# jakepoz/rnnt

Hardware: AMD Instinct MI355X
Metric: RNN-T joint+loss fwd+bwd lattice cells/s (B*T*U/s) (higher is better)
Workload: dtype f32(f16x2); 1 GPU; cfg2: B=32,T=1000,U=200,H=512,V=1024 fp32-class (f16x2 arithmetic) joint+loss fwd+bwd; enc_layout=contiguous (B,T,H), global_batch=32, per_gpu_batch=32, parallelism=dp1, cells_BTU1=6432000

## Files before the change

### rnnt_amd/csrc/common.hpp

```cpp
#pragma once
#include <hip/hip_runtime.h>
#include <stdint.h>

typedef float f32x16 __attribute__((ext_vector_type(16)));
typedef float f32x4 __attribute__((ext_vector_type(4)));

#define RNNT_NEG_INF (-__builtin_inff())
#ifdef RNNT_ABLATE
#define RNNT_XP(flags, bit) ((flags) & (bit))
#else
#define RNNT_XP(flags, bit) (0)
#endif
#define RNNT_LOG2E 1.4426950408889634f

#ifdef RNNT_VMCNT0
#define RNNT_VMCNT(n) "s_waitcnt vmcnt(0)"
#else
#define RNNT_VMCNT(n) "s_waitcnt vmcnt(" #n ")"
#endif

__device__ __forceinline__ long skew_index(int b, int t, int u, int D, int U1)
{
    return ((long)b * D + (t + u)) * U1 + u;
}

__device__ __forceinline__ int len_t(const int32_t *logit_lens, int b, int T)
{
    const int v = logit_lens[b];
    return v < 1 ? 1 : (v > T ? T : v);
}
__device__ __forceinline__ int len_u(const int32_t *target_lens, int b, int U1)
{
    const int v = target_lens[b];
    return v < 0 ? 0 : (v > U1 - 1 ? U1 - 1 : v);
}

__device__ __forceinline__ void len_tu_uniform(const int32_t *logit_lens, const int32_t *target_lens, int b, int T, int U1,
                                               int &Tb, int &Ub)
{
    int x, y;
    const int32_t *pl = logit_lens + b, *pt = target_lens + b;
    asm volatile("s_load_dword %0, %2, 0x0\n\ts_load_dword %1, %3, 0x0\n\ts_waitcnt lgkmcnt(0)"
                 : "=&s"(x), "=&s"(y) : "s"(pl), "s"(pt) : "memory");
    Tb = x < 1 ? 1 : (x > T ? T : x);
    Ub = y < 0 ? 0 : (y > U1 - 1 ? U1 - 1 : y);
}

__device__ __forceinline__ float fast_tanh(float x)
{
    float e = __builtin_amdgcn_exp2f(x * (2.0f * RNNT_LOG2E));
    return 1.0f - 2.0f * __builtin_amdgcn_rcpf(e + 1.0f);
}

typedef float f32x2_t __attribute__((ext_vector_type(2)));
__device__ __forceinline__ f32x2_t fast_tanh2(f32x2_t x)
{
    const f32x2_t a = x * (2.0f * RNNT_LOG2E);
    f32x2_t e = {__builtin_amdgcn_exp2f(a[0]), __builtin_amdgcn_exp2f(a[1])};
    e += 1.0f;
    const f32x2_t r = {__builtin_amdgcn_rcpf(e[0]), __builtin_amdgcn_rcpf(e[1])};
    return 1.0f - 2.0f * r;
}
__device__ __forceinline__ f32x4 fast_tanh_sum4(f32x4 e, f32x4 p)
{
    const f32x2_t lo = fast_tanh2(__builtin_shufflevector(e, e, 0, 1) + __builtin_shufflevector(p, p, 0, 1));
    const f32x2_t hi = fast_tanh2(__builtin_shufflevector(e, e, 2, 3) + __builtin_shufflevector(p, p, 2, 3));
    return f32x4{lo[0], lo[1], hi[0], hi[1]};
}

__device__ __forceinline__ float half_max(float v)
{
#pragma unroll
    for (int m = 16; m >= 1; m >>= 1) v = fmaxf(v, __shfl_xor(v, m, 64));
    return v;
}
__device__ __forceinline__ float half_sum(float v)
{
#pragma unroll
    for (int m = 16; m >= 1; m >>= 1) v += __shfl_xor(v, m, 64);
    return v;
}

template <int CTRL, int ROW_MASK>
__device__ __forceinline__ float dpp_mov(float old, float v)
{
    return __int_as_float(__builtin_amdgcn_update_dpp(__float_as_int(old), __float_as_int(v), CTRL, ROW_MASK, 0xf, false));
}
__device__ __forceinline__ float half_bcast(float v, int half)
{
    const float lo = __int_as_float(__builtin_amdgcn_readlane(__float_as_int(v), 31));
    const float hi = __int_as_float(__builtin_amdgcn_readlane(__float_as_int(v), 63));
    return half ? hi : lo;
}
__device__ __forceinline__ float half_max_dpp(float v, int half)
{
    asm volatile("s_nop 1\n\tv_max_f32_dpp %0, %0, %0 quad_perm:[1,0,3,2] row_mask:0xf bank_mask:0xf\n\t"
                 "s_nop 1\n\tv_max_f32_dpp %0, %0, %0 quad_perm:[2,3,0,1] row_mask:0xf bank_mask:0xf\n\t"
                 "s_nop 1\n\tv_max_f32_dpp %0, %0, %0 row_ror:4 row_mask:0xf bank_mask:0xf\n\t"
                 "s_nop 1\n\tv_max_f32_dpp %0, %0, %0 row_ror:8 row_mask:0xf bank_mask:0xf"
                 : "+v"(v));
    v = fmaxf(v, dpp_mov<0x142, 0xa>(RNNT_NEG_INF, v));
    return half_bcast(v, half);
}
__device__ __forceinline__ float half_sum_dpp(float v, int half)
{
    asm volatile("s_nop 1\n\tv_add_f32_dpp %0, %0, %0 quad_perm:[1,0,3,2] row_mask:0xf bank_mask:0xf\n\t"
                 "s_nop 1\n\tv_add_f32_dpp %0, %0, %0 quad_perm:[2,3,0,1] row_mask:0xf bank_mask:0xf\n\t"
                 "s_nop 1\n\tv_add_f32_dpp %0, %0, %0 row_ror:4 row_mask:0xf bank_mask:0xf\n\t"
                 "s_nop 1\n\tv_add_f32_dpp %0, %0, %0 row_ror:8 row_mask:0xf bank_mask:0xf"
                 : "+v"(v));
    v += dpp_mov<0x142, 0xa>(0.f, v);
    return v;
}

struct __attribute__((aligned(16))) CellCoef {
    float c1;
    float sb;
    float se;
    int y;
};
```

### rnnt_amd/csrc/x2.hip

```cpp
#include "kernels.hpp"

typedef __attribute__((ext_vector_type(8))) _Float16 f16x8;
typedef __attribute__((ext_vector_type(2))) _Float16 f16x2;
typedef __attribute__((ext_vector_type(4))) unsigned u32x4;
typedef __attribute__((ext_vector_type(2))) unsigned u32x2;
typedef __attribute__((ext_vector_type(4))) int i32x4;
typedef __attribute__((address_space(3))) void *lds_vptr;
typedef float f2 __attribute__((ext_vector_type(2)));

#ifdef RNNT_STAMPS
#define X2_CLOCK_STAMP(SLOT)                                                                                               \
    do {                                                                                                                   \
        if (a.debug && blockIdx.x == 0 && blockIdx.y == 0 && blockIdx.z == 0 && threadIdx.x == 0) {                        \
            unsigned long long t_, r_;                                                                                     \
            asm volatile("s_memtime %0\n\ts_memrealtime %1\n\ts_waitcnt lgkmcnt(0)" : "=s"(t_), "=s"(r_)::"memory");      \
            a.debug[SLOT] = t_; a.debug[(SLOT) + 1] = r_;                                                                  \
        }                                                                                                                  \
    } while (0)
#else
#define X2_CLOCK_STAMP(SLOT) do {} while (0)
#endif

#define X2_SH 16384.0f
#define X2_INV_SH (1.0f / 16384.0f)
// ... 1315 lines not shown
        __builtin_amdgcn_raw_ptr_buffer_load_lds(wrs, dst, 16, wvo, so, 1024, 0);
    };
    const int lds0 = (int)(size_t)(lds_vptr)s_dr;
    const int wb = lds0 + 16 * lane;

    f32x16 acc[4][4];
#pragma unroll
    for (int m = 0; m < 4; ++m)
#pragma unroll
        for (int n = 0; n < 4; ++n)
#pragma unroll
            for (int r = 0; r < 16; ++r) acc[m][n][r] = 0.f;

    AFrag ar[4];
    aload(ar[0], 0); aload(ar[1], 1); aload(ar[2], 2);
    wdma(0, 0); wdma(1, 1);
    int wsl = 0;
    for (int c0 = 0; c0 < VC; c0 += 4) {
#pragma unroll
        for (int j = 0; j < 4; ++j) {
            const int c = c0 + j;
            asm volatile(RNNT_VMCNT(10) ::: "memory");
            x2_lds_barrier();
            const int ws = wb + wsl * XR2_WSLOT;
            u32x4 bh[4], bm[4];
#pragma unroll
            for (int n = 0; n < 4; ++n) asm volatile("ds_read_b128 %0, %1 offset:%2" : "=v"(bh[n]) : "v"(ws), "n"(n * 1024));
            asm volatile("s_waitcnt lgkmcnt(0)" : "+v"(bh[0]), "+v"(bh[1]), "+v"(bh[2]), "+v"(bh[3]) :: "memory");
            AFrag &ac = ar[j], &an = ar[(j + 3) & 3];
            const int cn = c + 3;
            const int o = 8 * ((cn < VC ? cn : VC - 1) >> 1) + 2 * ((cn < VC ? cn : VC - 1) & 1);
#pragma unroll
            for (int m = 0; m < 4; ++m) {
#pragma unroll
                for (int n = 0; n < 4; ++n) {
                    acc[m][n] = x2_mfma(ac.h[m], bh[n], acc[m][n]);
                    if (m == 0) asm volatile("ds_read_b128 %0, %1 offset:%2" : "=v"(bm[n]) : "v"(ws), "n"(4096 + n * 1024));
                    if (n == 1) an.h[m] = arow[m][o];
                    if (n == 3) an.m[m] = arow[m][o + 4];
                    __builtin_amdgcn_sched_barrier(0);
                }
            }
#pragma unroll
            for (int m = 0; m < 4; ++m)
#pragma unroll
                for (int n = 0; n < 4; ++n) {
                    acc[m][n] = x2_mfma(ac.m[m], bh[n], acc[m][n]);
                    __builtin_amdgcn_sched_barrier(0);
                }
            asm volatile("s_waitcnt lgkmcnt(0)" : "+v"(bm[0]), "+v"(bm[1]), "+v"(bm[2]), "+v"(bm[3]) :: "memory");
#pragma unroll
            for (int m = 0; m < 4; ++m)
#pragma unroll
                for (int n = 0; n < 4; ++n) {
                    acc[m][n] = x2_mfma(ac.h[m], bm[n], acc[m][n]);
                    if (m == 3 && n == 0) wdma(c + 2, (wsl + 2) & 3);
                    __builtin_amdgcn_sched_barrier(0);
                }
            wsl = (wsl + 1) & 3;
        }
    }
    asm volatile("s_waitcnt vmcnt(0)" ::: "memory");
    if (!wlive) return;

    const int colg = 512 * hp + 4 * i;
    const bool colok = colg < H;
    f32x4 pr[8];
#pragma unroll
    for (int r7 = 0; r7 < 8; ++r7) {
        const int u = u0 + 8 * (r7 >> 2) + (r7 & 3) + 4 * half;
        pr[r7] = (u < U1 && colok) ? *(const f32x4 *)(a.pred + ((long)b * U1 + u) * H + colg) : f32x4{0.f, 0.f, 0.f, 0.f};
    }
    const float unscale = 4.0f * a.db_rescale * a.scales[1];
    const long BTH = (long)a.B * T * H, BUH = (long)a.B * U1 * H;
    auto dfac_q = [](f2 x) {
        const f2 av = x * (2.0f * RNNT_LOG2E);
        const f2 w = {__builtin_amdgcn_exp2f(-__builtin_fabsf(av[0])), __builtin_amdgcn_exp2f(-__builtin_fabsf(av[1]))};
        const f2 e1 = w + 1.0f;
        const f2 r = {__builtin_amdgcn_rcpf(e1[0]), __builtin_amdgcn_rcpf(e1[1])};
        return (w * r) * r;
    };
    f2 psum2[8][2];
#pragma unroll
    for (int k = 0; k < 8; ++k) { psum2[k][0] = f2{0.f, 0.f}; psum2[k][1] = f2{0.f, 0.f}; }
#pragma unroll
    for (int m = 0; m < 4; ++m)
#pragma unroll
        for (int rh = 0; rh < 2; ++rh) {
            const int t = t0 + 2 * m + rh;
            const f32x4 er = (t < T && colok) ? *(const f32x4 *)(a.enc + (long)b * a.enc_sb + (long)t * a.enc_st + colg) : f32x4{0.f, 0.f, 0.f, 0.f};
            f2 esum2[2] = {f2{0.f, 0.f}, f2{0.f, 0.f}};
#pragma unroll
            for (int r7 = 0; r7 < 8; ++r7)
#pragma unroll
                for (int qq = 0; qq < 2; ++qq) {
                    const f2 x = {er[2 * qq] + pr[r7][2 * qq], er[2 * qq + 1] + pr[r7][2 * qq + 1]};
                    const f2 av = {acc[m][2 * qq][rh * 8 + r7], acc[m][2 * qq + 1][rh * 8 + r7]};
                    const f2 d = av * dfac_q(x);
                    esum2[qq] += d;
                    psum2[r7][qq] += d;
                }
            f32x4 es = {unscale * esum2[0][0], unscale * esum2[0][1], unscale * esum2[1][0], unscale * esum2[1][1]};
#pragma unroll
            for (int q = 0; q < 4; ++q) es[q] += __shfl_xor(es[q], 32, 64);
            if (half == 0 && t < Tb && colok) *(f32x4 *)(a.slab_enc + (long)ub * BTH + ((long)b * T + t) * H + colg) = es;
        }
#pragma unroll
    for (int k = 0; k < 8; ++k) {
        const int u = u0 + 8 * (k >> 2) + (k & 3) + 4 * half;
        if (u < U1 && colok) {
            const f32x4 o = {unscale * psum2[k][0][0], unscale * psum2[k][0][1], unscale * psum2[k][1][0], unscale * psum2[k][1][1]};
            *(f32x4 *)(a.slab_pred + (long)tt * BUH + ((long)b * U1 + u) * H + colg) = o;
        }
    }
}

#define XZ2_WG_WAVES 4
__global__ __launch_bounds__(64 * XZ2_WG_WAVES) void k_x2_dead_rows(X3Args a, int ntt, int nub)
{
    const int lane = threadIdx.x & 63;
    const long wave = (long)blockIdx.x * XZ2_WG_WAVES + (threadIdx.x >> 6), nwave = (long)gridDim.x * XZ2_WG_WAVES;
    const long cells = (long)a.B * a.T * a.U1;
    const bool by_ks = a.dw_ksteps;
    const int sh = by_ks ? 4 : 2, per = 64 >> sh;
    const int *list = by_ks ? a.ks_list : a.grp_list;
    const long n = a.live_stats[by_ks ? 0 : 4];
    const int V4 = a.V / 4;
    const u32x4 z = {0u, 0u, 0u, 0u};
    for (long k = per * wave; k < n; k += per * nwave) {
        const long kk = k + (lane >> sh);
        int e = 0;
        bool dead = false;
        if (kk < n) {
            e = list[kk];
            const long c = ((long)e << sh) + (lane & ((1 << sh) - 1));
            if (c < cells) {
                const int u = (int)(c % a.U1);
                const long bt = c / a.U1;
                const int t = (int)(bt % a.T);
                const long b = bt / a.T;
                dead = a.tile_live[(b * ntt + t / XG2_BT_) * nub + u / XG2_BU_] == 0;
            }
        }
        unsigned long long m = __ballot(dead);
        for (; m; m &= m - 1) {
            const int r = __builtin_ctzll(m);
            u32x4 *row = (u32x4 *)(a.logits + (((long)__shfl(e, r, 64) << sh) + (r & ((1 << sh) - 1))) * a.V);
            for (int q = lane; q < V4; q += 64) row[q] = z;
        }
    }
}
void launch_x2_dead_rows(const X3Args &a, hipStream_t st)
{
    const long rounds = ((long)a.B * a.T * a.U1 + 63) / 64;
    const long want = (rounds + XZ2_WG_WAVES - 1) / XZ2_WG_WAVES, cap = (long)(a.n_cu > 0 ? a.n_cu : 256) * 8;
    const int ntt = (a.T + XG2_BT_ - 1) / XG2_BT_;
    hipLaunchKernelGGL(k_x2_dead_rows, dim3((unsigned)(want < cap ? want : cap)), dim3(64 * XZ2_WG_WAVES), 0, st, a, ntt, a.n_ublk16);
}

bool x2_dhidden_ok(int U1, int H, int V)
{
    return (long)((XG2_BT - 1) * (long)U1 + XG2_BU) * V * 4 < 0x7fffffffL && V % 128 == 0 && H % 128 == 0;
}

void launch_dhidden_x2(const X3Args &a, hipStream_t st)
{
    static bool attr_set[16] = {false};
    int dev = -1;
    if (hipGetDevice(&dev) != hipSuccess || dev < 0 || dev >= 16) dev = -1;
    const int lds = XG2_NW * XG2_WSLOT + 2 * XG2_XSLOT;
    if (dev < 0 || !attr_set[dev]) {
        (void)hipFuncSetAttribute((const void *)k_dhidden_x2<true, false>, hipFuncAttributeMaxDynamicSharedMemorySize, lds);
        (void)hipFuncSetAttribute((const void *)k_dhidden_x2<false, false>, hipFuncAttributeMaxDynamicSharedMemorySize, lds);
        (void)hipFuncSetAttribute((const void *)k_dhidden_x2<true, true>, hipFuncAttributeMaxDynamicSharedMemorySize, lds);
        (void)hipFuncSetAttribute((const void *)k_dhidden_x2<false, true>, hipFuncAttributeMaxDynamicSharedMemorySize, lds);
        if (dev >= 0) attr_set[dev] = true;
    }
    dim3 grid((unsigned)((long)a.n_ublk16 * ((a.T + XG2_BT - 1) / XG2_BT) * a.B));
    if (a.H < 512) hipLaunchKernelGGL((k_dhidden_x2<true, true>), grid, dim3(256), lds, st, a, 0);
    else hipLaunchKernelGGL((k_dhidden_x2<true, false>), grid, dim3(256), lds, st, a, 0);
    for (int hp = 1; hp * 512 < a.H; ++hp) {
        if (a.H - 512 * hp == 128) {
            dim3 gr(a.n_ublk16, ((a.T + XG2_BT - 1) / XG2_BT + 3) / 4, a.B);
            hipLaunchKernelGGL(k_dhidden_x2r, gr, dim3(256), XR2_NW * XR2_WSLOT, st, a, hp);
        }
        else if (a.H - 512 * hp < 512) hipLaunchKernelGGL((k_dhidden_x2<false, true>), grid, dim3(256), lds, st, a, hp);
        else hipLaunchKernelGGL((k_dhidden_x2<false, false>), grid, dim3(256), lds, st, a, hp);
    }
}

__global__ __launch_bounds__(256) void k_x2_make_ep(X3Args a)
{
    const int H = a.H, H4 = H / 4, KC = H / 16;
    const long n_enc = (long)a.B * a.T * H4, n_all = n_enc + (long)a.B * a.U1 * H4;
    const long idx = (long)blockIdx.x * 256 + threadIdx.x;
    bool big = false;
    if (idx < n_all) {
        const bool is_enc = idx < n_enc;
        const long j = is_enc ? idx : idx - n_enc;
        const long row = j / H4;
        const int h = (int)(j - row * H4) * 4;
        const int R = is_enc ? a.T : a.U1;
        const int b = (int)(row / R), r = (int)(row - (long)b * R);
        const float *src = is_enc ? a.enc + (long)b * a.enc_sb + (long)r * a.enc_st + h : a.pred + row * H + h;
        const f32x4 x = *(const f32x4 *)src;
        f32x4 y;
#pragma unroll
        for (int k = 0; k < 4; ++k) {
            big = big || !(fabsf(x[k]) <= 43.0f);
            double arg = (double)x[k] * 2.8853900817779268;
            arg = arg > 126.0 ? 126.0 : (arg < -126.0 ? -126.0 : arg);
            y[k] = (float)exp2(arg);
        }
        float *dst = (is_enc ? a.ep_enc : a.ep_pred) + (((long)b * KC + (h >> 4)) * R + r) * 16 + (h & 15);
        *(f32x4 *)dst = y;
    }
    if (__builtin_amdgcn_ballot_w64(big) != 0 && (threadIdx.x & 63) == 0) atomicOr(a.ep_flag, 1u);
}
void launch_x2_make_ep(const X3Args &a, hipStream_t st)
{
    launch_fill32(a.ep_flag, 0u, 4, st);
    const long n = ((long)a.B * a.T + (long)a.B * a.U1) * (a.H / 4);
    hipLaunchKernelGGL(k_x2_make_ep, dim3((unsigned)((n + 255) / 256)), dim3(256), 0, st, a);
}
size_t x2_ep_bytes(int B, int T, int U1, int H) { return ((size_t)B * T + (size_t)B * U1) * H * 4; }

__global__ __launch_bounds__(256) void k_x2_pack_w_fwd(const float *__restrict__ W, const float *__restrict__ scales, u32x4 *__restrict__ out, int H, int V, long n)
{
    const long idx = (long)blockIdx.x * 256 + threadIdx.x;
    if (idx >= n) return;
    const int lane = (int)(idx & 63), tile = (int)(idx >> 6) & 15;
    const int KC = H / 16;
    const int c = (int)((idx >> 10) % KC), pass = (int)((idx >> 10) / KC);
    const int v = 512 * pass + 128 * (tile >> 2) + 4 * (lane & 31) + (tile & 3);
    const int h0 = 16 * c + 8 * (lane >> 5);
    const float sw = scales[0];
    u32x4 ph = {0u, 0u, 0u, 0u}, pm = ph;
    if (v < V) {
        const float *w = W + (long)v * H + h0;
        f32x4 w0 = *(const f32x4 *)w, w1 = *(const f32x4 *)(w + 4);
#pragma unroll
        for (int k = 0; k < 4; ++k) { w0[k] = x2_clamp(w0[k] * sw); w1[k] = x2_clamp(w1[k] * sw); }
        X2_SPLIT4(w0, ph, pm, 0);
        X2_SPLIT4(w1, ph, pm, 2);
    }
    u32x4 *o = out + ((long)pass * KC + c) * 2048 + tile * 64 + lane;
    o[0] = ph; o[1024] = pm;
}
size_t x2_wpack_fwd_bytes(int H, int V) { return (size_t)((V + 511) / 512) * (H / 16) * 2 * 16 * 64 * 16; }

#define XF2_WSLOT 32768
#define XF2_ASLOT 8192
#define XF2_NW 3
#ifdef RNNT_STAMPS
#ifndef X2S_WAVE
#define X2S_WAVE 0
#endif
#define X2STAMP(slot)                                                                                       \
    do {                                                                                                    \
        if (a.debug && blockIdx.x == 0 && wave == X2S_WAVE && lane == 0 && it == 1 && cs >= 8 && cs < 24) {  \
            unsigned long long t_;                                                                          \
            asm volatile("s_memtime %0\n\ts_waitcnt lgkmcnt(0)" : "=s"(t_)::"memory");                       \
            a.debug[(cs - 8) * 8 + (slot)] = t_;                                                            \
        }                                                                                                   \
    } while (0)
#else
#define X2STAMP(slot) do {} while (0)
#endif
template <int MODE>
__global__ __launch_bounds__(256, 1) void k_joint_fwd_x2(X3Args a, const int ntiles)
{
    constexpr bool EP = MODE == 1, LIN = MODE == 2;
    if (!LIN && (*a.ep_flag != 0) == EP) return;
    extern __shared__ __attribute__((aligned(1024))) char s_fw[];
    float *s_den = (float *)(s_fw + XF2_NW * XF2_WSLOT + 2 * XF2_ASLOT);
    float *s_part = s_den + 128;
    int *s_next = (int *)(s_part + 512);
    const int tid = threadIdx.x, lane = tid & 63;
    const int wave = __builtin_amdgcn_readfirstlane(tid >> 6);
    const int wm = wave >> 1, wn = wave & 1;
    const int i = lane & 31, half = lane >> 5;
    const int H = a.H, V = a.V, KC = H / 16, U1 = a.U1, T = a.T;
    const int npass = (V + 511) / 512;
    const int NS = LIN ? KC : npass * KC;
    const long cells = (long)a.B * T * U1;
    const float unscale = (LIN ? a.scales[3] : X2_INV_SH) * a.scales[1];
    const float sx = LIN ? a.scales[2] : 1.0f;

    const int lds0 = (int)(size_t)(lds_vptr)s_fw;
    const int xa = lds0 + XF2_NW * XF2_WSLOT + (2 * wm) * 2048 + 16 * lane;
    const int xw = lds0 + XF2_NW * XF2_WSLOT + wave * 2048 + 16 * lane;
    const int wb = lds0 + (8 * wn) * 1024 + 16 * lane;
    const __amdgpu_buffer_rsrc_t wrs = __builtin_amdgcn_make_buffer_rsrc(a.wpack_fwd, 0, npass * KC * XF2_WSLOT, 0x00020000);
    const int wvo = lane * 16;

    X2_CLOCK_STAMP(128 + 100);
    if (tid == 0) s_next[0] = (int)atomicAdd(a.counter, 1u);
    __syncthreads();
    int tile = s_next[0];
    for (int it = 1; tile < ntiles; ++it) {
        if (tid == 0) s_next[it & 1] = (int)atomicAdd(a.counter, 1u);
        const long row0 = (long)(LIN ? tile / npass : tile) * 128;
        const int pass0 = LIN ? tile % npass : 0, cs0 = pass0 * KC;
        for (int k = tid; k < 256; k += 256) { s_part[2 * k] = RNNT_NEG_INF; s_part[2 * k + 1] = 0.f; }
        __syncthreads();
        const int next = s_next[it & 1];
        bool dead = false;
        if (!LIN) {
            const long per = (long)T * U1, c_last = row0 + 127;
            const long b_first = row0 / per;
            dead = c_last < cells && c_last / per == b_first && (row0 - b_first * per) / U1 >= len_t(a.logit_lens, (int)b_first, T);
        }

        const long prow = row0 + 32 * wave + i;
        const long pc_ = prow < cells ? prow : cells - 1;
        const int pu = (int)(pc_ % U1);
        const long pbt = pc_ / U1;
        const int pt = (int)(pbt % T), pb = (int)(pbt / T);
        const float *ep = EP ? a.ep_enc + ((long)pb * KC * T + pt) * 16 + 8 * half : a.enc + (long)pb * a.enc_sb + (long)pt * a.enc_st + 8 * half;
        const float *pp = LIN ? ep : EP ? a.ep_pred + ((long)pb * KC * U1 + pu) * 16 + 8 * half : a.pred + ((long)pb * U1 + pu) * H + 8 * half;
        const long ek = EP ? (long)T * 16 : 16, pk = EP ? (long)U1 * 16 : 16;
        u32x4 *hdst = (u32x4 *)a.hidden + pc_ * (H / 8) + half;
        const long ps = a.plane_stride / 8;
        struct Opd { f32x4 e0, e1, p0, p1; };
        struct Prod { f2 w[4]; float ra, rb; u32x4 ph, pm; };
        auto op_load1 = [&](Opd &o, int kcs, int k) {
            const float *e = ep + ek * kcs, *q = pp + pk * kcs;
            if (k == 0) o.e0 = *(const f32x4 *)e;
            else if (k == 1) o.e1 = *(const f32x4 *)(e + 4);
            else if (LIN) return;
            else if (k == 2) o.p0 = *(const f32x4 *)q;
            else o.p1 = *(const f32x4 *)(q + 4);
        };
        auto op_load = [&](Opd &o, int kcs) {
#pragma unroll
            for (int k = 0; k < 4; ++k) op_load1(o, kcs, k);
        };
        auto prod_piece = [&](Prod &P, const Opd &o, auto off_c, int k) {
            if (k < 8) {
                const int j = k >> 1;
                const f32x4 &e = j < 2 ? o.e0 : o.e1, &pv = j < 2 ? o.p0 : o.p1;
                const int q = 2 * (j & 1);
                if (LIN) {
                    if (!(k & 1)) P.w[j] = f2{x2_clamp(e[q] * sx), x2_clamp(e[q + 1] * sx)};
                } else if (EP) {
                    if (!(k & 1)) {
                        P.w[j] = f2{__builtin_amdgcn_rcpf(fmaf(e[q], pv[q], 1.0f)), __builtin_amdgcn_rcpf(fmaf(e[q + 1], pv[q + 1], 1.0f))};
                    } else {
                        P.w[j] = f2{fmaf(-2.0f * X2_SH, P.w[j][0], X2_SH), fmaf(-2.0f * X2_SH, P.w[j][1], X2_SH)};
                    }
                } else if (!(k & 1)) {
                    const f2 x = {e[q] + pv[q], e[q + 1] + pv[q + 1]};
                    const f2 av = x * (2.0f * RNNT_LOG2E);
                    P.w[j] = f2{__builtin_amdgcn_exp2f(av[0]), __builtin_amdgcn_exp2f(av[1])};
                } else {
                    const f2 ex = P.w[j] + 1.0f;
                    const f2 rr = {__builtin_amdgcn_rcpf(ex[0]), __builtin_amdgcn_rcpf(ex[1])};
                    P.w[j] = X2_SH - (2.0f * X2_SH) * rr;
                }
            } else if (k < 16) {
                const int j = (k - 8) >> 1;
                if (!(k & 1)) {
                    const unsigned hh = x2_pack(P.w[j][0], P.w[j][1]);
                    P.ph[j] = hh;
                    asm("v_fma_mix_f32 %0, %1, -1.0, %2 op_sel_hi:[1,0,0]" : "=v"(P.ra) : "v"(hh), "v"(P.w[j][0]));
                    asm("v_fma_mix_f32 %0, %1, -1.0, %2 op_sel:[1,0,0] op_sel_hi:[1,0,0]" : "=v"(P.rb) : "v"(hh), "v"(P.w[j][1]));
                } else {
                    P.pm[j] = x2_pack(P.ra, P.rb);
                }
            } else {
                const int dst = xw;
                asm volatile("ds_write_b128 %0, %1 offset:%2" :: "v"(dst), "v"(P.ph), "n"(decltype(off_c)::value) : "memory");
                asm volatile("ds_write_b128 %0, %1 offset:%2" :: "v"(dst), "v"(P.pm), "n"(decltype(off_c)::value + 1024) : "memory");
            }
        };
        auto hid_store = [&](const Prod &P, int kcs) { hdst[2 * kcs] = P.ph; hdst[2 * kcs + ps] = P.pm; };
        auto wdma = [&](int cs, int slot, int n) {
            const int g4 = n & 4;
            if ((n & 3) == 0) __builtin_amdgcn_raw_ptr_buffer_load_lds(wrs, (lds_vptr)(s_fw + slot * XF2_WSLOT + (wave * 8 + g4) * 1024), 16, wvo, (cs * 32 + wave * 8 + g4) * 1024, 0, 0);
            if ((n & 3) == 1) __builtin_amdgcn_raw_ptr_buffer_load_lds(wrs, (lds_vptr)(s_fw + slot * XF2_WSLOT + (wave * 8 + g4) * 1024), 16, wvo, (cs * 32 + wave * 8 + g4) * 1024, 1024, 0);
            if ((n & 3) == 2) __builtin_amdgcn_raw_ptr_buffer_load_lds(wrs, (lds_vptr)(s_fw + slot * XF2_WSLOT + (wave * 8 + g4) * 1024), 16, wvo, (cs * 32 + wave * 8 + g4) * 1024, 2048, 0);
            if ((n & 3) == 3) __builtin_amdgcn_raw_ptr_buffer_load_lds(wrs, (lds_vptr)(s_fw + slot * XF2_WSLOT + (wave * 8 + g4) * 1024), 16, wvo, (cs * 32 + wave * 8 + g4) * 1024, 3072, 0);
        };

        if (dead) {
            for (int kc = 0; kc < KC; ++kc) {
                Opd o; Prod P;
                op_load(o, kc);
#pragma unroll
                for (int pc = 0; pc < 16; ++pc) prod_piece(P, o, X2Int<0>{}, pc);
                hid_store(P, kc);
            }
            tile = next;
            continue;
        }

        f32x16 acc[2][8];
        auto acc_init = [&]() {
#pragma unroll
            for (int mt = 0; mt < 2; ++mt)
#pragma unroll
                for (int q = 0; q < 8; ++q)
#pragma unroll
                    for (int r = 0; r < 16; ++r) acc[mt][q][r] = 0.f;
        };
        Opd oset[2];
        struct Frag { u32x4 af[2][2], bf[8]; };
        Frag fr[2];
        auto frag_read1 = [&](Frag &f, auto xs_c, const int wslot, const int n) {
            const int xs = xa, ws = wb + wslot * XF2_WSLOT;
            if (n < 4) asm volatile("ds_read_b128 %0, %1 offset:%2" : "=v"(f.af[(n >> 1) & 1][n & 1]) : "v"(xs), "n"(decltype(xs_c)::value + ((n >> 1) & 1) * 2048 + (n & 1) * 1024));
            else asm volatile("ds_read_b128 %0, %1 offset:%2" : "=v"(f.bf[n >= 4 ? n - 4 : 0]) : "v"(ws), "n"((n >= 4 ? n - 4 : 0) * 1024));
        };
        auto frag_read = [&](Frag &f, auto xs_c, const int wslot) {
#pragma unroll
            for (int n = 0; n < 12; ++n) frag_read1(f, xs_c, wslot, n);
        };
        auto frag_landed = [&](Frag &f) {
            asm volatile("s_waitcnt lgkmcnt(0)"
                         : "+v"(f.af[0][0]), "+v"(f.af[0][1]), "+v"(f.af[1][0]), "+v"(f.af[1][1]),
                           "+v"(f.bf[0]), "+v"(f.bf[1]), "+v"(f.bf[2]), "+v"(f.bf[3]), "+v"(f.bf[4]), "+v"(f.bf[5]), "+v"(f.bf[6]), "+v"(f.bf[7])
                         :: "memory");
        };
        {
#pragma unroll
            for (int n = 0; n < 8; ++n) wdma(cs0, 0, n);
#pragma unroll
            for (int n = 0; n < 8; ++n) wdma(cs0 + (NS > 1 ? 1 : 0), 1, n);
#pragma unroll
            for (int n = 0; n < 8; ++n) wdma(cs0 + (NS > 2 ? 2 : NS - 1), 2, n);
            Opd o; Prod P;
            op_load(oset[1], KC > 1 ? 1 : 0);
            op_load(o, 0);
#pragma unroll
            for (int pc = 0; pc < 17; ++pc) prod_piece(P, o, X2Int<0>{}, pc);
            if (!LIN) hid_store(P, 0);
            asm volatile("s_waitcnt vmcnt(0)" ::: "memory");
            x2_lds_barrier();
            frag_read(fr[0], X2Int<0>{}, 0);
            frag_landed(fr[0]);
        }

        int cs = 0, wsl = 0;
        auto run_pass = [&](auto store_c, const int pass) {
          acc_init();
          constexpr bool STORE = decltype(store_c)::value != 0;
          auto kstep = [&](auto par_c, const int kc) {
            constexpr int par = decltype(par_c)::value;
            constexpr int XN = (1 - par) * XF2_ASLOT;
            Frag &fc = fr[par], &fn = fr[1 - par];
            const int ws = wb + wsl * XF2_WSLOT;
            const int csn = cs0 + (cs + 3 < NS ? cs + 3 : NS - 1), kcn = kc + 1 < KC ? kc + 1 : 0, kcnn = kcn + 1 < KC ? kcn + 1 : 0;
            const int wsn = wsl == 2 ? 0 : wsl + 1;
            const Opd &ocur = oset[(par + 1) & 1];
            Opd &onext = oset[par & 1];
            Prod P;
            u32x4 bn[8];
            X2STAMP(0);
            auto block = [&](auto pa_c, const u32x4 (&bcur)[8], auto blk_c) {
                constexpr int PA = decltype(pa_c)::value, BLK = decltype(blk_c)::value;
#pragma unroll
                for (int q = 0; q < 8; ++q) {
                    acc[0][q] = x2_mfma(fc.af[0][PA], bcur[q], acc[0][q]);
                    acc[1][q] = x2_mfma(fc.af[1][PA], bcur[q], acc[1][q]);
                    if (BLK == 0) {
                        asm volatile("ds_read_b128 %0, %1 offset:%2" : "=v"(bn[q]) : "v"(ws), "n"(16384 + q * 1024));
                        prod_piece(P, ocur, X2Int<XN>{}, q);
                    }
                    if (BLK == 1) {
                        if (q < (LIN ? 2 : 4)) op_load1(onext, kcnn, q);
                        if (q < 4) { prod_piece(P, ocur, X2Int<XN>{}, 8 + 2 * q); prod_piece(P, ocur, X2Int<XN>{}, 9 + 2 * q); }
                        if (q == 4) prod_piece(P, ocur, X2Int<XN>{}, 16);
                    }
                    if (BLK == 2) {
                        if (q < 4) { frag_read1(fn, X2Int<XN>{}, wsn, 2 * q); frag_read1(fn, X2Int<XN>{}, wsn, 2 * q + 1); }
                        else frag_read1(fn, X2Int<XN>{}, wsn, 4 + q);
                        wdma(csn, wsl, q);
                        if (STORE && q == 6) hdst[2 * kcn] = P.ph;
                        if (STORE && q == 7) hdst[2 * kcn + ps] = P.pm;
                    }
                    __builtin_amdgcn_sched_barrier(0);
                }
            };
            block(X2Int<0>{}, fc.bf, X2Int<0>{});
            X2STAMP(1);
            block(X2Int<1>{}, fc.bf, X2Int<1>{});
            X2STAMP(2);
            if (kc >= 2) {
                constexpr int NV = LIN ? 12 : (STORE ? 4 : 0) + 4 + 8 + 4;
                static_assert(NV == 12 || NV == 16 || NV == 20, "counted vmcnt of the forward's k-step");
                if (NV == 12) asm volatile(RNNT_VMCNT(12) ::: "memory");
                else if (NV == 16) asm volatile(RNNT_VMCNT(16) ::: "memory");
                else asm volatile(RNNT_VMCNT(20) ::: "memory");
            }
            X2STAMP(3);
            x2_lds_barrier();
            X2STAMP(4);
            asm volatile("" : "+v"(bn[0]), "+v"(bn[1]), "+v"(bn[2]), "+v"(bn[3]), "+v"(bn[4]), "+v"(bn[5]), "+v"(bn[6]), "+v"(bn[7]));
            block(X2Int<0>{}, bn, X2Int<2>{});
            frag_landed(fn);
            X2STAMP(5);
            (void)kcn;
            ++cs;
            wsl = wsn;
          };
          for (int kc0 = 0; kc0 < KC; kc0 += 2) { kstep(X2Int<0>{}, kc0); kstep(X2Int<1>{}, kc0 + 1); }
          if (STORE) asm volatile(RNNT_VMCNT(2) ::: "memory");
          else asm volatile("s_waitcnt vmcnt(0)" ::: "memory");
          {
            const int cw = 512 * pass + 256 * wn;
            const unsigned lane_off = (unsigned)(((4 * half) * V + 4 * i) * 4);
            char *tile_base = (char *)(a.logits + row0 * V + cw);
            const bool has_b = !LIN || a.bias != nullptr;
            const f32x4 b0 = has_b && cw + 4 * i < V ? *(const f32x4 *)(a.bias + cw + 4 * i) : f32x4{0.f, 0.f, 0.f, 0.f};
            const f32x4 b1 = has_b && cw + 128 + 4 * i < V ? *(const f32x4 *)(a.bias + cw + 128 + 4 * i) : f32x4{0.f, 0.f, 0.f, 0.f};
            auto epilogue = [&](auto both_c) {
                constexpr bool BOTH = decltype(both_c)::value != 0;
                auto slot = [&](int mt, int r) {
                    f32x4 o0, o1;
#pragma unroll
                    for (int q = 0; q < 4; ++q) {
                        float x0, x1;
                        asm volatile("v_accvgpr_read_b32 %0, %1" : "=v"(x0) : "a"(acc[mt][q][r]));
                        asm volatile("v_accvgpr_read_b32 %0, %1" : "=v"(x1) : "a"(acc[mt][4 + q][r]));
                        o0[q] = fmaf(x0, unscale, b0[q]); o1[q] = fmaf(x1, unscale, b1[q]);
                    }
                    char *rowp = tile_base + (long)(32 * (2 * wm + mt) + (r & 3) + 8 * (r >> 2)) * V * 4;
                    if (LIN) {
                        if (row0 + 32 * (2 * wm + mt) + (r & 3) + 8 * (r >> 2) + 4 * half < cells) {
                            *(f32x4 *)(rowp + lane_off) = o0;
                            if (BOTH) *(f32x4 *)(rowp + lane_off + 512) = o1;
                        }
                        return;
                    }
                    __builtin_nontemporal_store(o0, (f32x4 *)(rowp + lane_off));
                    if (BOTH) __builtin_nontemporal_store(o1, (f32x4 *)(rowp + lane_off + 512));
                    float m8 = fmaxf(fmaxf(o0[0], o0[1]), fmaxf(o0[2], o0[3]));
                    if (BOTH) m8 = fmaxf(m8, fmaxf(fmaxf(o1[0], o1[1]), fmaxf(o1[2], o1[3])));
                    const float M = half_max_dpp(m8, half);
                    const float nm2 = -M * RNNT_LOG2E;
                    float e = (__builtin_amdgcn_exp2f(fmaf(o0[0], RNNT_LOG2E, nm2)) + __builtin_amdgcn_exp2f(fmaf(o0[1], RNNT_LOG2E, nm2))) +
                              (__builtin_amdgcn_exp2f(fmaf(o0[2], RNNT_LOG2E, nm2)) + __builtin_amdgcn_exp2f(fmaf(o0[3], RNNT_LOG2E, nm2)));
                    if (BOTH)
                        e += (__builtin_amdgcn_exp2f(fmaf(o1[0], RNNT_LOG2E, nm2)) + __builtin_amdgcn_exp2f(fmaf(o1[1], RNNT_LOG2E, nm2))) +
                             (__builtin_amdgcn_exp2f(fmaf(o1[2], RNNT_LOG2E, nm2)) + __builtin_amdgcn_exp2f(fmaf(o1[3], RNNT_LOG2E, nm2)));
                    const float S_ = half_sum_dpp(e, half);
                    if (i == 31) {
                        float *sp = s_part + (wn * 128 + 32 * (2 * wm + mt) + (r & 3) + 8 * (r >> 2) + 4 * half) * 2;
                        const float m_o = sp[0], s_o = sp[1];
                        const float mn = fmaxf(m_o, M);
                        sp[0] = mn;
                        sp[1] = s_o * __builtin_amdgcn_exp2f((m_o - mn) * RNNT_LOG2E) + S_ * __builtin_amdgcn_exp2f((M - mn) * RNNT_LOG2E);
                    }
                };
#pragma unroll
                for (int mt = 0; mt < 2; ++mt)
#pragma unroll
                    for (int r = 0; r < 16; r += 2) {
                        slot(mt, r);
                        slot(mt, r + 1);
                        __builtin_amdgcn_sched_barrier(0);
                    }
            };
            if (cw + 128 < V) epilogue(X2Int<1>{});
            else if (cw < V) epilogue(X2Int<0>{});
          }
        };
        run_pass(X2Int<(LIN ? 0 : 1)>{}, pass0);
        if (!LIN)
            for (int pass = 1; pass < npass; ++pass) run_pass(X2Int<0>{}, pass);

        asm volatile("s_waitcnt vmcnt(0)" ::: "memory");
        __syncthreads();
        if (LIN) { tile = next; continue; }
        if (tid < 128) {
            const float m0 = s_part[tid * 2], s0 = s_part[tid * 2 + 1];
            const float m1 = s_part[(128 + tid) * 2], s1 = s_part[(128 + tid) * 2 + 1];
            const float M = fmaxf(m0, m1);
            const float S_ = s0 * __builtin_amdgcn_exp2f((m0 - M) * RNNT_LOG2E) + s1 * __builtin_amdgcn_exp2f((m1 - M) * RNNT_LOG2E);
            s_den[tid] = M + __logf(S_);
        }
        __syncthreads();
        {
            const int row = tid & 127, which = tid >> 7;
            const long cell = row0 + row;
            if (cell < cells) {
                const int u = (int)(cell % U1);
                const long bt = cell / U1;
                const int t = (int)(bt % T), b = (int)(bt / T);
                const int Ub = len_u(a.target_lens, b, U1);
                if (t < len_t(a.logit_lens, b, T) && u <= Ub) {
                    const float den = s_den[row];
                    const float *lrow = a.logits + cell * V;
                    const long si = skew_index(b, t, u, a.D, U1);
                    if (which == 0) {
                        const float lb = __hip_atomic_load(lrow + a.blank, __ATOMIC_RELAXED, __HIP_MEMORY_SCOPE_AGENT);
                        a.denom_s[si] = den;
                        a.lpb_s[si] = lb - den;
                    } else {
                        float le = 0.f;
                        if (u < Ub) {
                            const int y = a.targets[(long)b * (U1 - 1) + u];
                            le = __hip_atomic_load(lrow + y, __ATOMIC_RELAXED, __HIP_MEMORY_SCOPE_AGENT) - den;
                        }
                        a.lpe_s[si] = le;
                    }
                }
            }
        }
        tile = next;
    }
    X2_CLOCK_STAMP(128 + 102);
}

bool x2_fwd_ok(int U1, int H, int V) { return H % 128 == 0 && V % 128 == 0 && (long)128 * H * 2 < 0x7fffffffL; }

void launch_joint_fwd_x2(const X3Args &a, hipStream_t st)
{
    static bool attr_set[16] = {false};
    int dev = -1;
    if (hipGetDevice(&dev) != hipSuccess || dev < 0 || dev >= 16) dev = -1;
    const int lds = XF2_NW * XF2_WSLOT + 2 * XF2_ASLOT + 128 * 4 + 2 * 128 * 2 * 4 + 16;
    if (dev < 0 || !attr_set[dev]) {
        (void)hipFuncSetAttribute((const void *)k_joint_fwd_x2<1>, hipFuncAttributeMaxDynamicSharedMemorySize, lds);
        (void)hipFuncSetAttribute((const void *)k_joint_fwd_x2<0>, hipFuncAttributeMaxDynamicSharedMemorySize, lds);
        (void)hipFuncSetAttribute((const void *)k_joint_fwd_x2<2>, hipFuncAttributeMaxDynamicSharedMemorySize, lds);
        if (dev >= 0) attr_set[dev] = true;
    }
    const long cells = (long)a.B * a.T * a.U1;
    const bool lin = (a.flags & X2_FLAG_LINEAR) != 0;
    const int ntiles = (int)((cells + 127) / 128) * (lin ? (a.V + 511) / 512 : 1);
    if (!lin) launch_fill32(a.counter, 0u, 4, st);
    const int nwg = ntiles < a.n_cu ? ntiles : a.n_cu;
    if (a.flags & X2_FLAG_LINEAR) { hipLaunchKernelGGL(k_joint_fwd_x2<2>, dim3((unsigned)nwg), dim3(256), lds, st, a, ntiles); return; }
    hipLaunchKernelGGL(k_joint_fwd_x2<1>, dim3((unsigned)nwg), dim3(256), lds, st, a, ntiles);
    hipLaunchKernelGGL(k_joint_fwd_x2<0>, dim3((unsigned)nwg), dim3(256), lds, st, a, ntiles);
}

void launch_x2_pack_w(const X3Args &a, float *scales, hipStream_t st)
{
    hipLaunchKernelGGL(k_x2_wscale, dim3(1), dim3(1024), 0, st, a.W, (long)a.V * a.H / 4, scales);
    const long nd = (long)((a.H + 511) / 512) * (a.V / 16) * 16 * 64;
    hipLaunchKernelGGL(k_x2_pack_w_dh, dim3((unsigned)((nd + 255) / 256)), dim3(256), 0, st, a.W, (const float *)scales, (u32x4 *)a.wpack_dh, a.H, a.V, nd);
    const long nf = (long)((a.V + 511) / 512) * (a.H / 16) * 16 * 64;
    hipLaunchKernelGGL(k_x2_pack_w_fwd, dim3((unsigned)((nf + 255) / 256)), dim3(256), 0, st, a.W, (const float *)scales, (u32x4 *)a.wpack_fwd, a.H, a.V, nf);
}


struct X2AbsArgs { const float *x[3]; long ld[3], rows[3]; int cols4[3]; };
__global__ __launch_bounds__(256) void k_x2_absmax(X2AbsArgs a, float *__restrict__ partial)
{
    __shared__ float s_m[4];
    const int t = blockIdx.y;
    const float *x = a.x[t];
    const long ld = a.ld[t], n = a.rows[t] * a.cols4[t];
    const int cols4 = a.cols4[t];
    float m = 0.f;
    bool bad = false;
    for (long idx = (long)blockIdx.x * 256 + threadIdx.x; idx < n; idx += (long)gridDim.x * 256) {
        const long r = idx / cols4;
        const int c = (int)(idx - r * cols4);
        const f32x4 w = *(const f32x4 *)(x + r * ld + 4 * c);
        const float mw = fmaxf(fmaxf(fabsf(w[0]), fabsf(w[1])), fmaxf(fabsf(w[2]), fabsf(w[3])));
        bad = bad || !(fabsf(w[0]) <= X2_F32_MAX) || !(fabsf(w[1]) <= X2_F32_MAX) || !(fabsf(w[2]) <= X2_F32_MAX) || !(fabsf(w[3]) <= X2_F32_MAX);
        m = fmaxf(m, mw);
    }
#pragma unroll
    for (int o = 32; o > 0; o >>= 1) m = fmaxf(m, __shfl_xor(m, o, 64));
    const int any_bad = __syncthreads_or(bad ? 1 : 0);
    if ((threadIdx.x & 63) == 0) s_m[threadIdx.x >> 6] = m;
    __syncthreads();
    if (threadIdx.x == 0) partial[t * 256 + blockIdx.x] = any_bad ? __uint_as_float(0x7fc00000u) : fmaxf(fmaxf(s_m[0], s_m[1]), fmaxf(s_m[2], s_m[3]));
}
__global__ __launch_bounds__(256) void k_x2_lin_scales(const float *__restrict__ partial, float *__restrict__ scales, int n, unsigned *__restrict__ zero0,
                                                       int nzero0, unsigned *__restrict__ zero1, int nzero1, long nks,
                                                       int *__restrict__ list, int *__restrict__ stats, int *__restrict__ glist)
{
    __shared__ float s_m[4];
    for (int i = 0; i < n; ++i) {
        float m = partial[i * 256 + threadIdx.x];
        const int nonfinite = __syncthreads_or(m != m ? 1 : 0);
#pragma unroll
        for (int o = 32; o > 0; o >>= 1) m = fmaxf(m, __shfl_xor(m, o, 64));
        __syncthreads();
        if ((threadIdx.x & 63) == 0) s_m[threadIdx.x >> 6] = m;
        __syncthreads();
        if (threadIdx.x == 0 && nonfinite) {
            scales[2 * i] = 1.0f;
            scales[2 * i + 1] = __uint_as_float(0x7fc00000u);
        } else if (threadIdx.x == 0) {
            const unsigned bits = __float_as_uint(fmaxf(fmaxf(s_m[0], s_m[1]), fmaxf(s_m[2], s_m[3])));
            float s = 1.0f;
            const int e = (int)(bits >> 23) & 0xff;
            if (e > 0 && e < 255) {
                int k = 14 - (e - 126);
                k = k > 100 ? 100 : (k < -100 ? -100 : k);
                s = __uint_as_float((unsigned)(127 + k) << 23);
            }
            scales[2 * i] = s;
            scales[2 * i + 1] = 1.0f / s;
        }
    }
    for (int j = threadIdx.x; j < nzero0; j += 256) zero0[j] = 0u;
    for (int j = threadIdx.x; j < nzero1; j += 256) zero1[j] = 0u;
    if (list) {
        const long ngrp = 4 * nks;
        for (long j = threadIdx.x; j < nks + 8; j += 256) list[j] = (int)(j < nks ? j : nks);
        for (long j = threadIdx.x; j < ngrp + XL2_GPAD; j += 256) glist[j] = (int)(j < ngrp ? j : ngrp);
        if (threadIdx.x == 0) { stats[0] = (int)nks; stats[1] = (int)nks; stats[2] = 0; stats[3] = 0; stats[4] = (int)ngrp; stats[5] = (int)ngrp; }
    }
}
template <bool INTER>
__global__ __launch_bounds__(256) void k_x2_split_rows(const float *__restrict__ x, long ld, long rows, long rows_out, int cols,
                                                       const float *__restrict__ scale, void *__restrict__ dst, long plane_stride)
{
    const float s = scale[0];
    const long idx = (long)blockIdx.x * 256 + threadIdx.x;
    if (INTER) {
        const int VC = cols / 32;
        if (idx >= rows_out * VC) return;
        const long r = idx / VC;
        const int c = (int)(idx - r * VC);
        const f32x4 *p = (const f32x4 *)(x + (r < rows ? r : 0) * ld + 32 * c);
        u32x4 ph[4], pm[4];
#pragma unroll
        for (int i = 0; i < 8; ++i) {
            f32x4 v = r < rows ? p[i] : f32x4{0.f, 0.f, 0.f, 0.f};
#pragma unroll
            for (int k = 0; k < 4; ++k) v[k] = x2_clamp(v[k] * s);
            X2_SPLIT4(v, ph[i >> 1], pm[i >> 1], 2 * (i & 1));
        }
        u32x4 *o = (u32x4 *)((float *)dst + r * cols + 32 * c);
#pragma unroll
        for (int i = 0; i < 4; ++i) { o[i] = ph[i]; o[4 + i] = pm[i]; }
    } else {
        const int H8 = cols / 8;
        if (idx >= rows_out * H8) return;
        const long r = idx / H8;
        const int h = (int)(idx - r * H8) * 8;
        const float *xr = x + (r < rows ? r : 0) * ld + h;
        f32x4 t0 = *(const f32x4 *)xr, t1 = *(const f32x4 *)(xr + 4);
        if (r >= rows) t0 = t1 = f32x4{0.f, 0.f, 0.f, 0.f};
#pragma unroll
        for (int k = 0; k < 4; ++k) { t0[k] = x2_clamp(t0[k] * s); t1[k] = x2_clamp(t1[k] * s); }
        u32x4 ph, pm;
        X2_SPLIT4(t0, ph, pm, 0);
        X2_SPLIT4(t1, ph, pm, 2);
        u32x4 *o = (u32x4 *)((unsigned short *)dst + r * cols + h);
        o[0] = ph; o[plane_stride / 8] = pm;
    }
}
__global__ __launch_bounds__(256) void k_x2_reduce_scaled(const float *__restrict__ slab, float *__restrict__ out, long n4, long stride4, int nsplit,
                                                          const float *__restrict__ sa, const float *__restrict__ sb)
{
    const long i = (long)blockIdx.x * 256 + threadIdx.x;
    if (i >= n4) return;
    f32x4 acc = ((const f32x4 *)slab)[i];
    for (int s = 1; s < nsplit; ++s) acc += ((const f32x4 *)slab)[i + s * stride4];
    const float r = sa[0] * (sb ? sb[0] : 1.0f);
    ((f32x4 *)out)[i] = acc * r;
}

namespace {
struct LinWs { size_t wt, pack, pa, pb, slab_w, slab_b, prog, list, glist, total; long rows_pad, rows_alloc; int n_split; };
LinWs lin_layout(int M, int K, int N, bool bwd)
{
    auto al = [](size_t x) { return (x + 255) & ~(size_t)255; };
    LinWs L{};
    size_t o = 4096;
    if (!bwd) { L.pack = o; o += al(x2_wpack_fwd_bytes(K, N)); L.total = o; return L; }
    L.rows_pad = ((long)M + 1 + 31) / 32 * 32;
    L.rows_alloc = (L.rows_pad + 96 + 127) / 128 * 128;
    const long tiles = x2_dw_tiles(K, N);
    long ns = 256 / tiles;
    if (ns < 1) ns = 1;
    if (ns > L.rows_pad / 32) ns = L.rows_pad / 32;
    L.n_split = (int)ns;
    L.wt = o; o += al((size_t)N * K * 4);
    L.pack = o; o += al(x2_wpack_fwd_bytes(N, K));
    L.pa = o; o += al((size_t)L.rows_alloc * N * 4);
    L.pb = o; o += al((size_t)L.rows_alloc * K * 4);
    L.slab_w = o; o += al((size_t)L.n_split * N * K * 4);
    L.slab_b = o; o += al((size_t)L.n_split * N * 4);
    L.prog = o; o += al((size_t)L.n_split * 64);
    L.list = o; o += al(64 + (size_t)(L.rows_pad / XW2_ROWS + 8) * 4);
    L.glist = o; o += al((size_t)(L.rows_pad / 4 + XL2_GPAD) * 4);
    L.total = o;
    return L;
}
int lin_cus()
{
    static thread_local int cus[16] = {0};
    int dev = 0;
    if (hipGetDevice(&dev) != hipSuccess || dev < 0 || dev >= 16) dev = 0;
    if (!cus[dev]) {
        hipDeviceProp_t p;
        if (hipGetDeviceProperties(&p, dev) == hipSuccess) cus[dev] = p.multiProcessorCount;
        if (cus[dev] <= 0) cus[dev] = 256;
    }
    return cus[dev];
}
struct LinT { const float *x; long ld, rows; int cols; };
void lin_scales(const LinT *t, int n, char *w, unsigned *zero1, int nzero1, long nks, int *list, int *glist, hipStream_t st)
{
    X2AbsArgs a{};
    for (int i = 0; i < n; ++i) { a.x[i] = t[i].x; a.ld[i] = t[i].ld; a.rows[i] = t[i].rows; a.cols4[i] = t[i].cols / 4; }
    float *partial = (float *)(w + 1024);
    hipLaunchKernelGGL(k_x2_absmax, dim3(256, n), dim3(256), 0, st, a, partial);
    hipLaunchKernelGGL(k_x2_lin_scales, dim3(1), dim3(256), 0, st, partial, (float *)w, n, (unsigned *)(w + 128), 16, zero1, nzero1, nks,
                       list ? list + 16 : nullptr, list, glist);
}
void lin_gemm_nt(const float *x, long ldx, const float *wmat, const float *bias, int M, int K, int N, float *y, const float *scales, void *pack,
                 unsigned *counter, hipStream_t st)
{
    const long nf = (long)((N + 511) / 512) * (K / 16) * 16 * 64;
    hipLaunchKernelGGL(k_x2_pack_w_fwd, dim3((unsigned)((nf + 255) / 256)), dim3(256), 0, st, wmat, scales, (u32x4 *)pack, K, N, nf);
    X3Args a{};
    a.enc = x; a.enc_sb = ldx; a.enc_st = 0; a.pred = nullptr; a.W = wmat; a.bias = bias;
    a.B = M; a.T = 1; a.U1 = 1; a.H = K; a.V = N; a.logits = y; a.wpack_fwd = pack; a.scales = scales;
    a.counter = counter; a.n_cu = lin_cus(); a.flags = X2_FLAG_LINEAR;
    launch_joint_fwd_x2(a, st);
}
}

size_t x2_linear_ws_bytes(int M, int K, int N, bool bwd) { return lin_layout(M, K, N, bwd).total; }
bool x2_linear_ok(int M, int K, int N) { return M > 0 && K % 128 == 0 && N % 128 == 0 && x2_fwd_ok(1, K, N) && x2_fwd_ok(1, N, K); }

void launch_linear_x2_fwd(const float *x, long ldx, const float *W, const float *bias, int M, int K, int N, float *y, void *ws, hipStream_t st)
{
    const LinWs L = lin_layout(M, K, N, false);
    char *w = (char *)ws;
    float *scales = (float *)w;
    const LinT t[2] = {{W, K, N, K}, {x, ldx, M, K}};
    lin_scales(t, 2, w, nullptr, 0, 0, nullptr, nullptr, st);
    lin_gemm_nt(x, ldx, W, bias, M, K, N, y, scales, w + L.pack, (unsigned *)(w + 128), st);
}

void launch_linear_x2_bwd(const float *x, long ldx, const float *W, const float *dy, int M, int K, int N, float *dx, float *dW, float *db, void *ws,
                          hipStream_t st)
{
    const LinWs L = lin_layout(M, K, N, true);
    char *w = (char *)ws;
    float *scales = (float *)w;
    const LinT t[3] = {{W, K, N, K}, {dy, N, M, N}, {x, ldx, M, K}};
    lin_scales(t, 3, w, (unsigned *)(w + L.prog), L.n_split * 16, L.rows_pad / XW2_ROWS, (int *)(w + L.list), (int *)(w + L.glist), st);
    if (dx) {
        float *wt = (float *)(w + L.wt);
        launch_copy_enc(W, 0, 1, K, wt, 1, K, N, st);
        lin_gemm_nt(dy, N, wt, nullptr, M, N, K, dx, scales, w + L.pack, (unsigned *)(w + 128), st);
    }
    float *pa = (float *)(w + L.pa);
    unsigned short *pb = (unsigned short *)(w + L.pb);
    {
        const long na = L.rows_alloc * (N / 32), nb = L.rows_alloc * (K / 8);
        hipLaunchKernelGGL(k_x2_split_rows<true>, dim3((unsigned)((na + 255) / 256)), dim3(256), 0, st, dy, (long)N, (long)M, L.rows_alloc, N, scales + 2, (void *)pa, 0L);
        hipLaunchKernelGGL(k_x2_split_rows<false>, dim3((unsigned)((nb + 255) / 256)), dim3(256), 0, st, x, ldx, (long)M, L.rows_alloc, K, scales + 4, (void *)pb,
                           L.rows_alloc * (long)K);
    }
    X3Args a{};
    a.logits = pa; a.hidden = pb; a.plane_stride = L.rows_alloc * (long)K; a.rows_pad = L.rows_pad; a.rows_alloc = L.rows_alloc;
    a.B = 1; a.T = 1; a.U1 = 1; a.H = K; a.V = N; a.n_split = L.n_split; a.dw_prog = (int *)(w + L.prog);
    a.slab_w = (float *)(w + L.slab_w); a.slab_b = (float *)(w + L.slab_b); a.dw_rescale = 1.0f; a.db_rescale = 1.0f; a.n_cu = lin_cus();
    a.live_stats = (int *)(w + L.list); a.ks_list = a.live_stats + 16; a.grp_list = (int *)(w + L.glist);
    launch_dw_x2(a, st, false);
    const long n4w = (long)N * K / 4, n4b = N / 4;
    hipLaunchKernelGGL(k_x2_reduce_scaled, dim3((unsigned)((n4w + 255) / 256)), dim3(256), 0, st, a.slab_w, dW, n4w, n4w, L.n_split,
                       (const float *)(scales + 3), (const float *)(scales + 5));
    if (db)
        hipLaunchKernelGGL(k_x2_reduce_scaled, dim3((unsigned)((n4b + 255) / 256)), dim3(256), 0, st, a.slab_b, db, n4b, n4b, L.n_split,
                           (const float *)(scales + 3), (const float *)nullptr);
}
```

Before: 167.4 million cells/s.

## Batch DPP row reductions four-wide and keep online softmax stats in registers

The per-row max and sum reductions in the joint epilogue are now done four rows at a time with interleaved DPP trees, so the s_nop hazard stalls are shared across independent chains. Per-row results are packed into one lane per row with writelane, and the running max/sum merge is kept in registers across passes instead of being read-modified-written in LDS. The LDS partials are written once at the end of the tile, and the per-tile LDS initialization is removed. This relies on every lane slot being written, and it uses more registers for the four buffered outputs.

```diff
diff --git a/rnnt_amd/csrc/common.hpp b/rnnt_amd/csrc/common.hpp
--- a/rnnt_amd/csrc/common.hpp
+++ b/rnnt_amd/csrc/common.hpp
@@ -113,6 +113,28 @@
     return v;
 }
 
+#define RNNT_DPP4_STEP(op, ctrl)                     \
+    op " %0, %0, %0 " ctrl " bank_mask:0xf\n\t"     \
+    op " %1, %1, %1 " ctrl " bank_mask:0xf\n\t"     \
+    op " %2, %2, %2 " ctrl " bank_mask:0xf\n\t"     \
+    op " %3, %3, %3 " ctrl " bank_mask:0xf\n\t"
+#define RNNT_DPP4_TREE(op)                                        \
+    "s_nop 1\n\t"                                                 \
+    RNNT_DPP4_STEP(op, "quad_perm:[1,0,3,2] row_mask:0xf")        \
+    RNNT_DPP4_STEP(op, "quad_perm:[2,3,0,1] row_mask:0xf")        \
+    RNNT_DPP4_STEP(op, "row_ror:4 row_mask:0xf")                  \
+    RNNT_DPP4_STEP(op, "row_ror:8 row_mask:0xf")                  \
+    RNNT_DPP4_STEP(op, "row_bcast:15 row_mask:0xa")               \
+    "s_nop 1"
+__device__ __forceinline__ void half_max_dpp_x4(float &a, float &b, float &c, float &d)
+{
+    asm volatile(RNNT_DPP4_TREE("v_max_f32_dpp") : "+v"(a), "+v"(b), "+v"(c), "+v"(d));
+}
+__device__ __forceinline__ void half_sum_dpp_x4(float &a, float &b, float &c, float &d)
+{
+    asm volatile(RNNT_DPP4_TREE("v_add_f32_dpp") : "+v"(a), "+v"(b), "+v"(c), "+v"(d));
+}
+
 struct __attribute__((aligned(16))) CellCoef {
     float c1;
     float sb;
diff --git a/rnnt_amd/csrc/x2.hip b/rnnt_amd/csrc/x2.hip
--- a/rnnt_amd/csrc/x2.hip
+++ b/rnnt_amd/csrc/x2.hip
@@ -1641,7 +1641,6 @@
         if (tid == 0) s_next[it & 1] = (int)atomicAdd(a.counter, 1u);
         const long row0 = (long)(LIN ? tile / npass : tile) * 128;
         const int pass0 = LIN ? tile % npass : 0, cs0 = pass0 * KC;
-        for (int k = tid; k < 256; k += 256) { s_part[2 * k] = RNNT_NEG_INF; s_part[2 * k + 1] = 0.f; }
         __syncthreads();
         const int next = s_next[it & 1];
         bool dead = false;
@@ -1735,6 +1734,7 @@
         }
 
         f32x16 acc[2][8];
+        float m_run = RNNT_NEG_INF, s_run = 0.f;
         auto acc_init = [&]() {
 #pragma unroll
             for (int mt = 0; mt < 2; ++mt)
@@ -1855,8 +1855,7 @@
             const f32x4 b1 = has_b && cw + 128 + 4 * i < V ? *(const f32x4 *)(a.bias + cw + 128 + 4 * i) : f32x4{0.f, 0.f, 0.f, 0.f};
             auto epilogue = [&](auto both_c) {
                 constexpr bool BOTH = decltype(both_c)::value != 0;
-                auto slot = [&](int mt, int r) {
-                    f32x4 o0, o1;
+                auto read_slot = [&](int mt, int r, f32x4 &o0, f32x4 &o1) {
 #pragma unroll
                     for (int q = 0; q < 4; ++q) {
                         float x0, x1;
@@ -1864,42 +1863,80 @@
                         asm volatile("v_accvgpr_read_b32 %0, %1" : "=v"(x1) : "a"(acc[mt][4 + q][r]));
                         o0[q] = fmaf(x0, unscale, b0[q]); o1[q] = fmaf(x1, unscale, b1[q]);
                     }
-                    char *rowp = tile_base + (long)(32 * (2 * wm + mt) + (r & 3) + 8 * (r >> 2)) * V * 4;
-                    if (LIN) {
+                };
+                auto row_of = [&](int mt, int r) { return 32 * (2 * wm + mt) + (r & 3) + 8 * (r >> 2); };
+                if constexpr (LIN) {
+                    auto slot = [&](int mt, int r) {
+                        f32x4 o0, o1;
+#pragma unroll
+                        for (int q = 0; q < 4; ++q) {
+                            float x0, x1;
+                            asm volatile("v_accvgpr_read_b32 %0, %1" : "=v"(x0) : "a"(acc[mt][q][r]));
+                            asm volatile("v_accvgpr_read_b32 %0, %1" : "=v"(x1) : "a"(acc[mt][4 + q][r]));
+                            o0[q] = fmaf(x0, unscale, b0[q]); o1[q] = fmaf(x1, unscale, b1[q]);
+                        }
+                        char *rowp = tile_base + (long)(32 * (2 * wm + mt) + (r & 3) + 8 * (r >> 2)) * V * 4;
                         if (row0 + 32 * (2 * wm + mt) + (r & 3) + 8 * (r >> 2) + 4 * half < cells) {
                             *(f32x4 *)(rowp + lane_off) = o0;
                             if (BOTH) *(f32x4 *)(rowp + lane_off + 512) = o1;
                         }
-                        return;
-                    }
-                    __builtin_nontemporal_store(o0, (f32x4 *)(rowp + lane_off));
-                    if (BOTH) __builtin_nontemporal_store(o1, (f32x4 *)(rowp + lane_off + 512));
-                    float m8 = fmaxf(fmaxf(o0[0], o0[1]), fmaxf(o0[2], o0[3]));
-                    if (BOTH) m8 = fmaxf(m8, fmaxf(fmaxf(o1[0], o1[1]), fmaxf(o1[2], o1[3])));
-                    const float M = half_max_dpp(m8, half);
-                    const float nm2 = -M * RNNT_LOG2E;
-                    float e = (__builtin_amdgcn_exp2f(fmaf(o0[0], RNNT_LOG2E, nm2)) + __builtin_amdgcn_exp2f(fmaf(o0[1], RNNT_LOG2E, nm2))) +
-                              (__builtin_amdgcn_exp2f(fmaf(o0[2], RNNT_LOG2E, nm2)) + __builtin_amdgcn_exp2f(fmaf(o0[3], RNNT_LOG2E, nm2)));
-                    if (BOTH)
-                        e += (__builtin_amdgcn_exp2f(fmaf(o1[0], RNNT_LOG2E, nm2)) + __builtin_amdgcn_exp2f(fmaf(o1[1], RNNT_LOG2E, nm2))) +
-                             (__builtin_amdgcn_exp2f(fmaf(o1[2], RNNT_LOG2E, nm2)) + __builtin_amdgcn_exp2f(fmaf(o1[3], RNNT_LOG2E, nm2)));
-                    const float S_ = half_sum_dpp(e, half);
-                    if (i == 31) {
-                        float *sp = s_part + (wn * 128 + 32 * (2 * wm + mt) + (r & 3) + 8 * (r >> 2) + 4 * half) * 2;
-                        const float m_o = sp[0], s_o = sp[1];
-                        const float mn = fmaxf(m_o, M);
-                        sp[0] = mn;
-                        sp[1] = s_o * __builtin_amdgcn_exp2f((m_o - mn) * RNNT_LOG2E) + S_ * __builtin_amdgcn_exp2f((M - mn) * RNNT_LOG2E);
-                    }
-                };
-#pragma unroll
-                for (int mt = 0; mt < 2; ++mt)
-#pragma unroll
-                    for (int r = 0; r < 16; r += 2) {
-                        slot(mt, r);
-                        slot(mt, r + 1);
-                        __builtin_amdgcn_sched_barrier(0);
-                    }
+                    };
+#pragma unroll
+                    for (int mt = 0; mt < 2; ++mt)
+#pragma unroll
+                        for (int r = 0; r < 16; r += 2) {
+                            slot(mt, r);
+                            slot(mt, r + 1);
+                            __builtin_amdgcn_sched_barrier(0);
+                        }
+                } else {
+                    int m_pass = 0, s_pass = 0;
+#pragma unroll
+                    for (int mt = 0; mt < 2; ++mt)
+#pragma unroll
+                        for (int r0 = 0; r0 < 16; r0 += 4) {
+                            f32x4 o0[4], o1[4];
+                            float mx[4], sm[4];
+#pragma unroll
+                            for (int g = 0; g < 4; ++g) {
+                                read_slot(mt, r0 + g, o0[g], o1[g]);
+                                char *rowp = tile_base + (long)row_of(mt, r0 + g) * V * 4;
+                                __builtin_nontemporal_store(o0[g], (f32x4 *)(rowp + lane_off));
+                                if (BOTH) __builtin_nontemporal_store(o1[g], (f32x4 *)(rowp + lane_off + 512));
+                                float m8 = fmaxf(fmaxf(o0[g][0], o0[g][1]), fmaxf(o0[g][2], o0[g][3]));
+                                if (BOTH) m8 = fmaxf(m8, fmaxf(fmaxf(o1[g][0], o1[g][1]), fmaxf(o1[g][2], o1[g][3])));
+                                mx[g] = m8;
+                            }
+                            half_max_dpp_x4(mx[0], mx[1], mx[2], mx[3]);
+#pragma unroll
+                            for (int g = 0; g < 4; ++g) {
+                                const int lo = __builtin_amdgcn_readlane(__float_as_int(mx[g]), 31), hi = __builtin_amdgcn_readlane(__float_as_int(mx[g]), 63);
+                                asm("v_writelane_b32 %0, %1, %2" : "+v"(m_pass) : "s"(lo), "n"(16 * mt + r0 + g));
+                                asm("v_writelane_b32 %0, %1, %2" : "+v"(m_pass) : "s"(hi), "n"(32 + 16 * mt + r0 + g));
+                                const float M = __int_as_float(half ? hi : lo);
+                                const float nm2 = -M * RNNT_LOG2E;
+                                float e = (__builtin_amdgcn_exp2f(fmaf(o0[g][0], RNNT_LOG2E, nm2)) + __builtin_amdgcn_exp2f(fmaf(o0[g][1], RNNT_LOG2E, nm2))) +
+                                          (__builtin_amdgcn_exp2f(fmaf(o0[g][2], RNNT_LOG2E, nm2)) + __builtin_amdgcn_exp2f(fmaf(o0[g][3], RNNT_LOG2E, nm2)));
+                                if (BOTH)
+                                    e += (__builtin_amdgcn_exp2f(fmaf(o1[g][0], RNNT_LOG2E, nm2)) + __builtin_amdgcn_exp2f(fmaf(o1[g][1], RNNT_LOG2E, nm2))) +
+                                         (__builtin_amdgcn_exp2f(fmaf(o1[g][2], RNNT_LOG2E, nm2)) + __builtin_amdgcn_exp2f(fmaf(o1[g][3], RNNT_LOG2E, nm2)));
+                                sm[g] = e;
+                            }
+                            half_sum_dpp_x4(sm[0], sm[1], sm[2], sm[3]);
+#pragma unroll
+                            for (int g = 0; g < 4; ++g) {
+                                const int lo = __builtin_amdgcn_readlane(__float_as_int(sm[g]), 31), hi = __builtin_amdgcn_readlane(__float_as_int(sm[g]), 63);
+                                asm("v_writelane_b32 %0, %1, %2" : "+v"(s_pass) : "s"(lo), "n"(16 * mt + r0 + g));
+                                asm("v_writelane_b32 %0, %1, %2" : "+v"(s_pass) : "s"(hi), "n"(32 + 16 * mt + r0 + g));
+                            }
+                            __builtin_amdgcn_sched_barrier(0);
+                        }
+                    const float M = __int_as_float(m_pass), S_ = __int_as_float(s_pass);
+                    const float m_o = m_run, s_o = s_run;
+                    const float mn = fmaxf(m_o, M);
+                    m_run = mn;
+                    s_run = fmaf(s_o, __builtin_amdgcn_exp2f((m_o - mn) * RNNT_LOG2E), S_ * __builtin_amdgcn_exp2f((M - mn) * RNNT_LOG2E));
+                }
             };
             if (cw + 128 < V) epilogue(X2Int<1>{});
             else if (cw < V) epilogue(X2Int<0>{});
@@ -1909,6 +1946,11 @@
         if (!LIN)
             for (int pass = 1; pass < npass; ++pass) run_pass(X2Int<0>{}, pass);
 
+        if (!LIN) {
+            float *sp = s_part + (wn * 128 + 32 * (2 * wm + (i >> 4)) + (i & 3) + 8 * ((i & 15) >> 2) + 4 * half) * 2;
+            sp[0] = m_run;
+            sp[1] = s_run;
+        }
         asm volatile("s_waitcnt vmcnt(0)" ::: "memory");
         __syncthreads();
         if (LIN) { tile = next; continue; }
```

Result: faster. 169.5 million cells/s, median of 6 (+1.3%).
